# lukifer23/Matrix0

Measured on AMD Instinct MI355X. Metric: self-play games/sec at 800 sims/move, ResNet-24 53M; 1/2/4/8 MI355X, higher is better.
Workload: dtype f16

## Files before the change

### matrix0_amd/csrc/conv_gemm.hip

```cpp
#include "kernel_common.h"
#include "conv_epilogue.h"

template <int TAPS, int WN, int NT, int KC, ConvEpi EPI = EPI_ELEMENT, int ACT = ACT_NONE>
__global__ __launch_bounds__(256 * WN) void conv_gemm_kernel(GemmArgs a) {
    constexpr int NB = WN * NT * 32;
    constexpr int NTHR = 256 * WN;
    constexpr int AST = KC + 8;
    constexpr int APIX = (TAPS == 9) ? 100 : 64;
    constexpr int A_ELEMS = 4 * APIX * AST;
    constexpr int W_ELEMS = NB * AST;
    constexpr int A_PIECES = 4 * 64 * KC / 8;
    constexpr int W_PIECES = NB * KC / 8;
    constexpr int A_PER = (A_PIECES + NTHR - 1) / NTHR;
    constexpr int W_PER = (W_PIECES + NTHR - 1) / NTHR;
    constexpr int K8 = KC / 8;

    extern __shared__ __attribute__((aligned(16))) char smem[];
    _Float16* A_lds = reinterpret_cast<_Float16*>(smem);
    _Float16* W_lds = A_lds + A_ELEMS;

    const int tid = threadIdx.x;
    const int lane = tid & 63;
    const int wave = tid >> 6;
    const int wm = wave % 4;
    const int wn = wave / 4;
    const int m0 = blockIdx.x * 256;
    const int n0 = blockIdx.y * NB;
    const int Cin = a.Cin;
    const int nchunk = Cin / KC;
    const int Npad = a.Npad;

    if (TAPS == 9) {
        for (int i = tid; i < A_ELEMS / 8; i += NTHR)
            reinterpret_cast<uint4*>(A_lds)[i] = make_uint4(0, 0, 0, 0);
    }
    __syncthreads();

    float16v acc[2][NT];
    static_for<0, 2>([&](auto mi) __attribute__((always_inline)) {
        static_for<0, NT>([&](auto ni) __attribute__((always_inline)) {
            acc[decltype(mi)::value][decltype(ni)::value] = float16v{0.f, 0.f, 0.f, 0.f, 0.f, 0.f, 0.f, 0.f,
                                                                      0.f, 0.f, 0.f, 0.f, 0.f, 0.f, 0.f, 0.f};
        });
    });

    int apix[2];
#pragma unroll
    for (int mi = 0; mi < 2; ++mi) {
        int px = mi * 32 + (lane & 31);
        if (TAPS == 9) apix[mi] = wm * 100 + ((px >> 3) + 1) * 10 + (px & 7) + 1;
        else apix[mi] = wm * 64 + px;
    }
    const int khalf = 8 * (lane >> 5);

    uint4 areg[A_PER];
    uint4 wreg[W_PER];

    auto load_A = [&](int chunk) {
#pragma unroll
        for (int i = 0; i < A_PER; ++i) {
            int p = tid + i * NTHR;
            if (A_PIECES % NTHR == 0 || p < A_PIECES) {
                int row = p / K8, c8 = p % K8;
                areg[i] = *reinterpret_cast<const uint4*>(a.in + (size_t)(m0 + row) * Cin + chunk * KC + c8 * 8);
            }
        }
    };
    auto store_A = [&](int chunk) {
#pragma unroll
        for (int i = 0; i < A_PER; ++i) {
            int p = tid + i * NTHR;
            if (A_PIECES % NTHR == 0 || p < A_PIECES) {
                int row = p / K8, c8 = p % K8;
                int b = row >> 6, px = row & 63;
                uint4 v = areg[i];
                int pix = (TAPS == 9) ? (b * 100 + ((px >> 3) + 1) * 10 + (px & 7) + 1) : row;
                *reinterpret_cast<uint4*>(A_lds + pix * AST + c8 * 8) = v;
            }
        }
    };
    auto load_W = [&](int step) {
        int chunk = step / TAPS, tap = step % TAPS;
        const _Float16* src = a.w + ((size_t)(tap * nchunk + chunk) * Npad + n0) * KC;
#pragma unroll
        for (int i = 0; i < W_PER; ++i) {
            int p = tid + i * NTHR;
            if (W_PIECES % NTHR == 0 || p < W_PIECES)
                wreg[i] = *reinterpret_cast<const uint4*>(src + (size_t)p * 8);
        }
    };
    auto store_W = [&](int buf) {
#pragma unroll
        for (int i = 0; i < W_PER; ++i) {
            int p = tid + i * NTHR;
            if (W_PIECES % NTHR == 0 || p < W_PIECES) {
                int n = p / K8, k8 = p % K8;
                *reinterpret_cast<uint4*>(W_lds + buf * W_ELEMS + n * AST + k8 * 8) = wreg[i];
            }
        }
    };

    const int nsteps = nchunk * TAPS;
    load_A(0);
    load_W(0);
    for (int s = 0; s < nsteps; ++s) {
        const int chunk = s / TAPS, tap = s % TAPS;
        if (tap == 0) {
            if (s > 0) __syncthreads();
            store_A(chunk);
        }
        store_W(s & 1);
        __syncthreads();
        if (s + 1 < nsteps) {
            load_W(s + 1);
            if ((s + 1) % TAPS == 0) load_A((s + 1) / TAPS);
        }
        const int tapoff = (TAPS == 9) ? ((tap / 3 - 1) * 10 + (tap % 3 - 1)) : 0;
        const _Float16* Wb = W_lds + (s & 1) * W_ELEMS + (wn * NT * 32 + (lane & 31)) * AST + khalf;
        static_for<0, KC / 16>([&](auto kk_) __attribute__((always_inline)) {
            constexpr int kk = decltype(kk_)::value;
            half8 af0 = *reinterpret_cast<const half8*>(A_lds + (apix[0] + tapoff) * AST + kk * 16 + khalf);
            half8 af1 = *reinterpret_cast<const half8*>(A_lds + (apix[1] + tapoff) * AST + kk * 16 + khalf);
            static_for<0, NT>([&](auto ni_) __attribute__((always_inline)) {
                constexpr int ni = decltype(ni_)::value;
                half8 bf = *reinterpret_cast<const half8*>(Wb + ni * 32 * AST + kk * 16);
                acc[0][ni] = __builtin_amdgcn_mfma_f32_32x32x16_f16(af0, bf, acc[0][ni], 0, 0, 0);
                acc[1][ni] = __builtin_amdgcn_mfma_f32_32x32x16_f16(af1, bf, acc[1][ni], 0, 0, 0);
            });
        });
    }

    if constexpr (EPI == EPI_GN) {
        __syncthreads();
        GemmArgs o = a;
        int out_col0 = 0;
        if (a.out2 != nullptr && n0 + wn * NT * 32 >= a.nsplit) { o.out = a.out2; o.ldo = a.ldo2; out_col0 = a.nsplit; }
        conv_tile_epilogue<EPI_GN, ACT, NT>(acc, o, smem + wave * (64 * 64 * NT), m0, n0, wm, wn, lane, out_col0);
    } else {
        conv_tile_epilogue<EPI_ELEMENT, ACT_NONE, NT>(acc, a, smem, m0, n0, wm, wn, lane);
    }
}

template <int TAPS, int WN, int NT, int KC>
static size_t conv_gemm_lds() {
    constexpr int NB = WN * NT * 32;
    constexpr int AST = KC + 8;
    constexpr int APIX = (TAPS == 9) ? 100 : 64;
    const size_t main_loop = (size_t)(4 * APIX * AST + 2 * NB * AST) * 2 + 64;
    const size_t staging = (size_t)WN * 4 * 64 * 64 * NT;
    return main_loop > staging ? main_loop : staging;
}

template <int TAPS, int WN, int NT, int KC, ConvEpi EPI = EPI_ELEMENT, int ACT = ACT_NONE>
static hipError_t launch_conv_gemm_t(const GemmArgs& a, hipStream_t st) {
    constexpr int NB = WN * NT * 32;
    size_t lds = conv_gemm_lds<TAPS, WN, NT, KC>();
    static DeviceOnce once;
    hipError_t e = once.run([] {
        return hipFuncSetAttribute(reinterpret_cast<const void*>(&conv_gemm_kernel<TAPS, WN, NT, KC, EPI, ACT>),
                                   hipFuncAttributeMaxDynamicSharedMemorySize, 160 * 1024);
    });
    if (e != hipSuccess) return e;
    dim3 grid(a.Mrows / 256, a.Npad / NB);
    hipLaunchKernelGGL((conv_gemm_kernel<TAPS, WN, NT, KC, EPI, ACT>), grid, dim3(256 * WN), lds, st, a);
    return hipGetLastError();
}
template <int ACT>
static hipError_t launch_conv_gemm_gn(const GemmArgs& a, int taps, hipStream_t st) {
    if (a.bias != nullptr || a.mul != nullptr || a.out_stats != nullptr || a.out_f32 || a.out_scale != 1.f || a.Npad != a.N)
        return hipErrorInvalidValue;
    if (taps == 9) return a.Npad % 64 == 0 && a.out2 == nullptr ? launch_conv_gemm_t<9, 1, 2, 32, EPI_GN, ACT>(a, st) : hipErrorInvalidValue;
    if (a.posenc != nullptr) return hipErrorInvalidValue;
    if (a.out2 != nullptr) return a.Npad == 192 && a.nsplit == 64 ? launch_conv_gemm_t<1, 3, 2, 32, EPI_GN, ACT>(a, st) : hipErrorInvalidValue;
    if (a.Npad == 160) return launch_conv_gemm_t<1, 1, 5, 32, EPI_GN, ACT>(a, st);
    if (a.Npad == 128) return launch_conv_gemm_t<1, 2, 2, 32, EPI_GN, ACT>(a, st);
    if (a.Npad == 64) return launch_conv_gemm_t<1, 1, 2, 32, EPI_GN, ACT>(a, st);
    if (a.Npad == 32) return launch_conv_gemm_t<1, 1, 1, 32, EPI_GN, ACT>(a, st);
    return hipErrorInvalidValue;
}

hipError_t launch_conv_big(const GemmArgs& a, int taps, hipStream_t st);
hipError_t launch_conv_zs(const GemmArgs& a, hipStream_t st);

int conv_gemm_tile_n(int Cin, int Npad) {
    return (Npad % 320 == 0 && Cin % 64 == 0) ? 320 : 32;
}
int conv_gemm_kc(int Cin, int Npad) {
    return (Npad % 320 == 0 && Cin % 64 == 0) ? 64 : 32;
}

hipError_t launch_conv_gemm(const GemmArgs& a, int taps, hipStream_t st) {
    if (a.Mrows % 256 != 0 || a.Cin % 32 != 0 || a.Npad % 32 != 0) return hipErrorInvalidValue;
    const bool big = conv_gemm_tile_n(a.Cin, a.Npad) == 320;
    if (a.gn_gamma != nullptr && !big) {
        if (a.epi_act == ACT_SILU) return launch_conv_gemm_gn<ACT_SILU>(a, taps, st);
        if (a.epi_act == ACT_RELU) return launch_conv_gemm_gn<ACT_RELU>(a, taps, st);
        return hipErrorInvalidValue;
    }
    if (taps == 9) {
        if (big) {
            if (!a.w_pp) return hipErrorInvalidValue;
            return launch_conv_zs(a, st);
        }
        return launch_conv_gemm_t<9, 1, 1, 32>(a, st);
    } else if (taps == 1) {
        if (big) return a.w_pp ? hipErrorInvalidValue : launch_conv_big(a, 1, st);
        if (a.Mrows / 256 >= 256 && a.Npad % 64 == 0) return launch_conv_gemm_t<1, 1, 2, 32>(a, st);
        return launch_conv_gemm_t<1, 1, 1, 32>(a, st);
    }
    return hipErrorInvalidValue;
}
```

### matrix0_amd/csrc/net.h

```cpp
#pragma once
#include <hip/hip_runtime.h>
#include <stdint.h>
#include <map>
#include <string>
#include <vector>
#include "../../include/m0_engine.h"
#include "net_kernels.h"

struct HostTensor {
    std::vector<float> data;
    std::vector<int64_t> shape;
};

struct PackedGemm {
    _Float16* w = nullptr;
    float* bias = nullptr;
    int taps = 1, Cin = 0, N = 0;
    bool pp = false;
};

struct NormParams {
    float* gamma = nullptr;
    float* beta = nullptr;
};

struct ResBlockW {
    PackedGemm conv1, conv2;
    NormParams bn1, bn2;
    float *se_w1 = nullptr, *se_b1 = nullptr, *se_w2 = nullptr, *se_b2 = nullptr;
    void* se_wf = nullptr;
    int se_hidden = 0;
};

struct AttnW {
    PackedGemm qkv, proj;
    NormParams ln;
    float* rel_bias = nullptr;
    void* blk_w = nullptr;
    _Float16* blk_bias = nullptr;
};

struct TowerLayer {
    int kind;
    int index;
    bool skip;
    int next_bn1 = -1;
};

struct SslHeadW {
    PackedGemm c0, c1;
    NormParams n;
    int out_ch = 0;
};

struct ConvNormOpts {
    const float* posenc = nullptr;
    const _Float16* res = nullptr;
    const NormParams* next_bn1 = nullptr;
};

class Net {
public:
    explicit Net(const m0_net_cfg& cfg, int device, hipStream_t stream);
    ~Net();
    Net* shared_view(hipStream_t stream) const;
    static const char* check_supported(const m0_net_cfg& cfg);
    int load(const char* name, const void* data, int dtype, const int64_t* shape, int ndim, std::string& err);
    int finalize(std::string& err);
    bool ready() const { return finalized_; }
    const std::vector<void*>& device_buffers() const { return dev_allocs_; }
    const std::vector<size_t>& device_buffer_bytes() const { return dev_sizes_; }

    int forward(const float* planes_dev, const _Float16* nhwc_dev, int B, float* logits_dev, float* value_dev,
                float* ssl_dev, hipStream_t st, std::string& err);
    int ensure_workspace(int B, std::string& err);
    int ssl_channels_total() const;
    const m0_net_cfg& cfg() const { return cfg_; }
    size_t param_count() const { return nparams_; }
    double flops_per_position(bool with_ssl) const;
    _Float16* input_nhwc() { return X0_; }
    void set_profile(bool on) { profile_ = on; }
    void harvest_profile();
    double prof_conv_ms() const { return prof_ms_; }
    double prof_conv_flop() const { return prof_flop_; }
    long prof_conv_launches() const { return prof_launches_; }
    void reset_profile() { prof_ms_ = 0; prof_flop_ = 0; prof_launches_ = 0; prof_tail_ms_ = 0; prof_tail_launches_ = 0; }
    double prof_tail_ms() const { return prof_tail_ms_; }
    long prof_tail_launches() const { return prof_tail_launches_; }

private:
    m0_net_cfg cfg_;
    int device_;
    hipStream_t stream_ = nullptr;
    struct Switches { bool fuse_tail = true, fuse_attn = true; int attn_grid = 0; } sw_;
    struct Plan {
        bool fuse_tail = false;
        bool fuse_attn = false;
        bool gn_small = false;
        int act = 0, vact = 0;
        int first_bn1 = -1;
    } plan_;
    bool finalized_ = false;
    size_t nparams_ = 0;
    std::map<std::string, HostTensor> sd_;
    std::vector<void*> dev_allocs_;
    std::vector<size_t> dev_sizes_;
    std::vector<void*> ws_allocs_;

    int C_ = 0, Cs_ = 0 ;
    int Cp_ = 0;
    PackedGemm stem_;
    NormParams stem_n_;
    float* posenc_ = nullptr;
    PackedGemm pst_, inter_;
    NormParams pst_n_, inter_n_;
    std::vector<ResBlockW> res_;
    std::vector<AttnW> att_;
    std::vector<TowerLayer> tower_;
    PackedGemm ph_conv_, pfc1_, pfc2_;
    PackedGemm hv_;
    NormParams hv_n_;
    NormParams ph_n_;
    float logit_scale_ = 1.f;
    PackedGemm vh0_, vh3_, vfc1_, vfc2_, vgate_, vfc3_;
    NormParams vh1_n_, vh4_n_;
    std::vector<SslHeadW> ssl_;
    uint64_t* mask_dev_ = nullptr;

    bool profile_ = false;
    std::vector<hipEvent_t> pev_;
    std::vector<double> pflop_;
    std::vector<char> ptail_;
    size_t pev_used_ = 0;
    double prof_ms_ = 0, prof_flop_ = 0, prof_tail_ms_ = 0;
    long prof_launches_ = 0, prof_tail_launches_ = 0;

    int wsB_ = 0, wsM_ = 0;
    _Float16 *X0_ = nullptr, *XA_ = nullptr, *XB_ = nullptr, *T1_ = nullptr, *T2_ = nullptr, *QKV_ = nullptr,
             *O_ = nullptr, *AA_ = nullptr;
    float *S1_ = nullptr, *S2_ = nullptr, *G_ = nullptr;
    _Float16 *PH_ = nullptr, *PH2_ = nullptr, *VH_ = nullptr, *VH2_ = nullptr, *F1_ = nullptr, *F2_ = nullptr,
             *F3_ = nullptr, *F4_ = nullptr, *SH_ = nullptr, *SH2_ = nullptr, *SO_ = nullptr;
    float* VAL_ = nullptr;
    float* SPK_ = nullptr;

    const HostTensor* get(const std::string& k, std::string& err);
    int pack_gemm(PackedGemm& g, const std::string& wkey, const std::string& bkey, int taps, int Cin_real,
                  int Cin_pad, int N_real, int N_pad, int k_perm_ch, std::string& err, int qkv_heads = 0,
                  int qkv_heads_pad = 0);
    int pack_attn_block(AttnW& a, const std::string& prefix, std::string& err);
    int pack_chess_features(std::string& err);
    int pack_se(ResBlockW& r, const std::string& prefix, std::string& err);
    int pack_attn(AttnW& a, bool skip, const std::string& prefix, std::string& err);
    void upload_attn_mask();
    int pack_joint_head(std::string& err);
    int pack_ssl_heads(std::string& err);
    void make_plan();
    int upload_norm(NormParams& n, const std::string& prefix, int C_real, int C_pad, std::string& err);
    float* upload_f32(const std::vector<float>& v);
    void* dalloc(size_t bytes, bool ws);
    const NormParams* bn1(int res_index) const { return res_index < 0 ? nullptr : &res_[res_index].bn1; }
    template <class Launch>
    hipError_t profiled(bool on, hipStream_t st, double flop, bool tail, Launch&& launch);
    hipError_t run_gemm(const PackedGemm& g, GemmArgs a, hipStream_t st);
    hipError_t conv_norm_act(const PackedGemm& g, const NormParams& n, const _Float16* in, _Float16* out, _Float16* scratch,
                             int Mrows, hipStream_t st, const ConvNormOpts& o = ConvNormOpts());
    hipError_t se_gate(const ResBlockW& r, const float* stats, int boards, hipStream_t st);
};
```

### matrix0_amd/csrc/net.hip

```cpp
#include "net.h"
#include "attn_math.h"
#include <math.h>
#include <string.h>
#include <algorithm>
#include <stdlib.h>

static inline int ceil_to(int v, int m) { return (v + m - 1) / m * m; }

static const char* kSslNames[5] = {"piece", "threat", "pin", "fork", "control"};
static const int kSslOut[5] = {13, 1, 1, 1, 3};

const char* Net::check_supported(const m0_net_cfg& c) {
    if (!c.norm_group) return "HIP path supports norm='group' only (BatchNorm configs are not built)";
    if (!c.preact) return "HIP path supports preact=true only";
    if (c.channels % 32 != 0 || c.channels < 32 || c.channels > 384) return "channels must be a multiple of 32 in [32,384]";
    if (c.planes < 1 || c.planes > 32) return "planes must be in [1,32]";
    if (c.attention && (c.attention_heads <= 0 || c.channels % c.attention_heads != 0 ||
                        c.channels / c.attention_heads != 16))
        return "attention head_dim (channels/attention_heads) must be 16";
    if (c.activation != M0_ACT_SILU && c.activation != M0_ACT_RELU) return "activation must be silu or relu";
    if (c.blocks < 1) return "blocks must be >= 1";
    if (c.policy_factor_rank < 0) return "policy_factor_rank must be >= 0";
    if (c.self_supervised && c.ssl_tasks && (c.channels / 2) % 16 != 0) return "ssl heads need channels/2 % 16 == 0";
    return nullptr;
}

Net::Net(const m0_net_cfg& cfg, int device, hipStream_t stream) : cfg_(cfg), device_(device), stream_(stream) {
    auto off = [](const char* name) { const char* e = getenv(name); return e && e[0] == '0'; };
    sw_.fuse_tail = !off("M0_FUSE_TAIL");
    sw_.fuse_attn = !off("M0_FUSE_ATTN");
    if (const char* e = getenv("M0_ATTN_GRID")) sw_.attn_grid = std::max(0, atoi(e));
    C_ = cfg.channels;
    Cp_ = (C_ > 256 && C_ < 320) ? 320 : C_;
    Cs_ = ceil_to(std::max(16, C_ / 2), 32);
    int k = cfg.attention_every_k;
    int stride = std::max(1, cfg.infer_attention_stride);
    int att_seen = 0;
    for (int i = 0; i < cfg.blocks; ++i) {
        tower_.push_back({0, (int)res_.size(), false});
        res_.emplace_back();
        if (cfg.attention && k > 0 && (i % k) == (k - 1)) {
            ++att_seen;
            bool skip = stride > 1 && (att_seen % stride) != 0;
            tower_.push_back({1, (int)att_.size(), skip});
            att_.emplace_back();
        }
    }
}

Net* Net::shared_view(hipStream_t stream) const {
    Net* v = new Net(*this);
    v->stream_ = stream;
    v->dev_allocs_.clear(); v->dev_sizes_.clear();
    v->ws_allocs_.clear(); v->wsB_ = 0; v->wsM_ = 0;
    v->sd_.clear();
    v->pev_.clear(); v->pflop_.clear(); v->ptail_.clear(); v->pev_used_ = 0; v->profile_ = false;
    v->prof_ms_ = v->prof_flop_ = v->prof_tail_ms_ = 0; v->prof_launches_ = v->prof_tail_launches_ = 0;
    return v;
}

Net::~Net() {
    for (hipEvent_t e : pev_) (void)hipEventDestroy(e);
    for (void* p : dev_allocs_) (void)hipFree(p);
    for (void* p : ws_allocs_) (void)hipFree(p);
}

void* Net::dalloc(size_t bytes, bool ws) {
    void* p = nullptr;
    if (bytes == 0) bytes = 16;
    if (hipMalloc(&p, bytes) != hipSuccess) return nullptr;
    (void)hipMemsetAsync(p, 0, bytes, stream_);
    if (!ws) (void)hipStreamSynchronize(stream_);
    (ws ? ws_allocs_ : dev_allocs_).push_back(p);
    if (!ws) dev_sizes_.push_back(bytes);
    return p;
}

float* Net::upload_f32(const std::vector<float>& v) {
    float* d = (float*)dalloc(v.size() * 4, false);
    if (d && !v.empty()) (void)hipMemcpy(d, v.data(), v.size() * 4, hipMemcpyHostToDevice);
    return d;
}

int Net::load(const char* name, const void* data, int dtype, const int64_t* shape, int ndim, std::string& err) {
    if (finalized_) { err = "weights already finalized"; return M0_ERR_STATE; }
    if (!name || (!data && ndim >= 0)) { err = "null argument"; return M0_ERR_INVALID; }
    HostTensor t;
    size_t n = 1;
    for (int i = 0; i < ndim; ++i) { t.shape.push_back(shape[i]); n *= (size_t)shape[i]; }
    t.data.resize(n);
    if (dtype == 0) memcpy(t.data.data(), data, n * 4);
    else if (dtype == 1) {
        const _Float16* h = (const _Float16*)data;
        for (size_t i = 0; i < n; ++i) t.data[i] = (float)h[i];
    } else { err = "dtype must be 0 (f32) or 1 (f16)"; return M0_ERR_INVALID; }
    std::string key(name);
    if (cfg_.policy_factor_rank > 0 && key.rfind("policy_fc.", 0) == 0) key = "policy_fc1." + key.substr(10);
    sd_[key] = std::move(t);
    return M0_OK;
}

const HostTensor* Net::get(const std::string& k, std::string& err) {
    auto it = sd_.find(k);
    if (it == sd_.end()) { err = "missing state-dict key: " + k; return nullptr; }
    return &it->second;
}

int Net::pack_gemm(PackedGemm& g, const std::string& wkey, const std::string& bkey, int taps, int Cin_real,
                   int Cin_pad, int N_real, int N_pad, int k_perm_ch, std::string& err, int qkv_heads, int qkv_heads_pad) {
    const HostTensor* w = get(wkey, err);
    if (!w) return M0_ERR_INVALID;
    size_t expect = (size_t)N_real * Cin_real * taps;
    if (w->data.size() != expect) { err = "shape mismatch for " + wkey; return M0_ERR_INVALID; }
    nparams_ += expect;
    const int KC = conv_gemm_kc(Cin_pad, N_pad);
    const int nchunk = Cin_pad / KC;
    const bool pp = KC == 64 && taps == 9;
    const int nblk = N_pad / 320;
    std::vector<_Float16> p((size_t)taps * Cin_pad * N_pad, (_Float16)0.f);
    for (int nr = 0; nr < N_real; ++nr)
        for (int k = 0; k < Cin_real; ++k)
            for (int t = 0; t < taps; ++t) {
                float v = w->data[((size_t)nr * Cin_real + k) * taps + t];
                int n = nr;
                if (qkv_heads > 0) {
                    const int d = nr % 16, th = nr / 16, hh = th % qkv_heads, tt = th / qkv_heads;
                    n = (tt * qkv_heads_pad + hh) * 16 + d;
                }
                int kk = k;
                if (k_perm_ch > 0) {
                    int c = k / 64, sq = k % 64;
                    kk = sq * k_perm_ch + c;
                }
                int chunk = kk / KC, kc = kk % KC;
                if (pp) {
                    const int kt = chunk * 9 + t, by = n / 320, nl = n % 320, h = kc >> 5, k32 = kc & 31;
                    const int kx = (((k32 >> 3) ^ ((4 - ((nl >> 2) & 3)) & 3)) << 3) | (k32 & 7);
                    p[((((size_t)kt * nblk + by) * 2 + h) * 320 + nl) * 32 + kx] = (_Float16)v;
                    continue;
                }
                if (KC == 64)
                    kc = (((kc >> 3) ^ ((n >> 1) & 7)) << 3) | (kc & 7);
                p[(((size_t)t * nchunk + chunk) * N_pad + n) * KC + kc] = (_Float16)v;
            }
    g.w = (_Float16*)dalloc(p.size() * 2, false);
    if (!g.w) { err = "hipMalloc failed"; return M0_ERR_HIP; }
    (void)hipMemcpy(g.w, p.data(), p.size() * 2, hipMemcpyHostToDevice);
    g.taps = taps; g.Cin = Cin_pad; g.N = N_pad; g.pp = pp;
    g.bias = nullptr;
    if (!bkey.empty()) {
        const HostTensor* b = get(bkey, err);
        if (!b) return M0_ERR_INVALID;
        if ((int)b->data.size() != N_real) { err = "shape mismatch for " + bkey; return M0_ERR_INVALID; }
        nparams_ += N_real;
        std::vector<float> bp(N_pad, 0.f);
        std::copy(b->data.begin(), b->data.end(), bp.begin());
        g.bias = upload_f32(bp);
    }
    return M0_OK;
}

int Net::pack_attn_block(AttnW& a, const std::string& prefix, std::string& err) {
    const HostTensor* wq = get(prefix + ".qkv.weight", err); if (!wq) return M0_ERR_INVALID;
    const HostTensor* wp = get(prefix + ".proj.weight", err); if (!wp) return M0_ERR_INVALID;
    const int Cr = C_, Hr = cfg_.attention_heads;
    if (Cp_ != 320 || Cr != Hr * 16 || wq->data.size() != (size_t)3 * Cr * Cr || wp->data.size() != (size_t)Cr * Cr) {
        err = "shape mismatch for " + prefix; return M0_ERR_INVALID;
    }
    std::vector<_Float16> buf(attn_block_pack_bytes() / 2, (_Float16)0.f);
    auto qkv_w = [&](int type, int h, int d, int k) -> float {
        return (h < Hr && k < Cr) ? wq->data[(size_t)((type * Hr + h) * 16 + d) * Cr + k] : 0.f;
    };
    auto proj_w = [&](int oc, int h, int d) -> float {
        return (oc < Cr && h < Hr) ? wp->data[(size_t)oc * Cr + h * 16 + d] : 0.f;
    };
    for (int g = 0; g < 10; ++g) {
        for (int pc = 0; pc < 5; ++pc) {
            const size_t base = (size_t)(g * 7 + pc) * 6144;
            for (int col = 0; col < 96; ++col) {
                const int J = col >> 4, type = J >> 1, hl = J & 1, d = col & 15;
                for (int k = 0; k < 64; ++k) {
                    const int pos = (k >> 3) ^ ((col >> 1) & 7);
                    buf[base + (size_t)col * 64 + pos * 8 + (k & 7)] = (_Float16)qkv_w(type, 2 * g + hl, d, 64 * pc + k);
                }
            }
        }
        for (int hh = 0; hh < 2; ++hh) {
            const size_t base = (size_t)(g * 7 + 5 + hh) * 6144;
            for (int cl = 0; cl < 160; ++cl)
                for (int k = 0; k < 32; ++k) {
                    const int pos = (k >> 3) ^ ((4 - ((cl >> 2) & 3)) & 3);
                    buf[base + (size_t)cl * 32 + pos * 8 + (k & 7)] = (_Float16)proj_w(160 * hh + cl, 2 * g + (k >> 4), k & 15);
                }
        }
    }
    a.blk_w = dalloc(buf.size() * 2, false);
    if (!a.blk_w) { err = "hipMalloc failed"; return M0_ERR_HIP; }
    (void)hipMemcpy(a.blk_w, buf.data(), buf.size() * 2, hipMemcpyHostToDevice);
    std::vector<_Float16> bb((size_t)20 * 2 * 64 * 32, (_Float16)0.f);
    if (cfg_.attention_relbias) {
        const HostTensor* rb = get(prefix + ".rel_bias", err); if (!rb) return M0_ERR_INVALID;
// ... 84 lines not shown
                    for (int e = 0; e < 8; ++e) {
                        const int j = 32 * ks + 8 * (l >> 4) + e, c = 16 * nt + (l & 15);
                        if (j < hd) wf[((size_t)(10 * NT1 + nt * KS2 + ks) * 64 + l) * 8 + e] = (_Float16)w2t[(size_t)j * P + c];
                    }
        r.se_wf = dalloc(wf.size() * 2, false);
        if (!r.se_wf) { err = "hipMalloc failed"; return M0_ERR_HIP; }
        (void)hipMemcpy(r.se_wf, wf.data(), wf.size() * 2, hipMemcpyHostToDevice);
    }
    std::vector<float> b2p(P, 0.f);
    std::copy(b2->data.begin(), b2->data.end(), b2p.begin());
    r.se_b2 = upload_f32(b2p);
    return M0_OK;
}

int Net::pack_attn(AttnW& a, bool skip, const std::string& p, std::string& err) {
    const int C = C_, P = Cp_;
    if (skip) {
        for (const char* k : {".qkv.weight", ".proj.weight", ".norm.weight", ".norm.bias", ".rel_bias"}) {
            auto it = sd_.find(p + k);
            if (it != sd_.end()) nparams_ += it->second.data.size();
        }
        return M0_OK;
    }
    TRY(pack_gemm(a.qkv, p + ".qkv.weight", "", 1, C, P, 3 * C, 3 * P, 0, err, P != C ? cfg_.attention_heads : 0, P / 16));
    TRY(pack_gemm(a.proj, p + ".proj.weight", "", 1, C, P, C, P, 0, err));
    TRY(upload_norm(a.ln, p + ".norm", C, P, err));
    if (P == 320) TRY(pack_attn_block(a, p, err));
    if (cfg_.attention_relbias) {
        const HostTensor* rb = get(p + ".rel_bias", err); if (!rb) return M0_ERR_INVALID;
        if ((int)rb->data.size() != cfg_.attention_heads * 4096) { err = "shape mismatch for rel_bias"; return M0_ERR_INVALID; }
        nparams_ += rb->data.size();
        std::vector<float> rbs((size_t)(P / 16) * 4096, 0.f);
        for (size_t i = 0; i < rb->data.size(); ++i) rbs[i] = rb->data[i] * kLog2e;
        a.rel_bias = upload_f32(rbs);
    }
    return M0_OK;
}

void Net::upload_attn_mask() {
    std::vector<uint64_t> m(64, 0);
    for (int i = 0; i < 64; ++i)
        for (int j = 0; j < 64; ++j) {
            int dr = i / 8 - j / 8, dc = i % 8 - j % 8;
            int adr = abs(dr), adc = abs(dc);
            bool vis = dr == 0 || dc == 0 || adr == adc || (adr == 2 && adc == 1) || (adr == 1 && adc == 2) ||
                       (adr <= 1 && adc <= 1);
            if (vis) m[i] |= (1ull << j);
        }
    mask_dev_ = (uint64_t*)dalloc(64 * 8, false);
    (void)hipMemcpy(mask_dev_, m.data(), 64 * 8, hipMemcpyHostToDevice);
}

int Net::pack_joint_head(std::string& err) {
    const int nch = Cp_ / 32;
    std::vector<_Float16> a((size_t)nch * 64 * 32), b((size_t)nch * 128 * 32), c((size_t)nch * 192 * 32);
    (void)hipMemcpy(a.data(), ph_conv_.w, a.size() * 2, hipMemcpyDeviceToHost);
    (void)hipMemcpy(b.data(), vh0_.w, b.size() * 2, hipMemcpyDeviceToHost);
    for (int ch = 0; ch < nch; ++ch) {
        std::copy(a.begin() + (size_t)ch * 64 * 32, a.begin() + (size_t)(ch + 1) * 64 * 32, c.begin() + (size_t)ch * 192 * 32);
        std::copy(b.begin() + (size_t)ch * 128 * 32, b.begin() + (size_t)(ch + 1) * 128 * 32, c.begin() + ((size_t)ch * 192 + 64) * 32);
    }
    hv_.w = (_Float16*)dalloc(c.size() * 2, false);
    if (!hv_.w) { err = "hipMalloc failed"; return M0_ERR_HIP; }
    (void)hipMemcpy(hv_.w, c.data(), c.size() * 2, hipMemcpyHostToDevice);
    hv_.taps = 1; hv_.Cin = Cp_; hv_.N = 192; hv_.pp = false; hv_.bias = nullptr;
    std::vector<float> g(192), be(192);
    (void)hipMemcpy(g.data(), ph_n_.gamma, 64 * 4, hipMemcpyDeviceToHost);
    (void)hipMemcpy(g.data() + 64, vh1_n_.gamma, 128 * 4, hipMemcpyDeviceToHost);
    (void)hipMemcpy(be.data(), ph_n_.beta, 64 * 4, hipMemcpyDeviceToHost);
    (void)hipMemcpy(be.data() + 64, vh1_n_.beta, 128 * 4, hipMemcpyDeviceToHost);
    hv_n_.gamma = upload_f32(g); hv_n_.beta = upload_f32(be);
    if (!hv_n_.gamma || !hv_n_.beta) { err = "hipMalloc failed"; return M0_ERR_HIP; }
    return M0_OK;
}

int Net::pack_ssl_heads(std::string& err) {
    for (int t = 0; t < 5; ++t) {
        if (!(cfg_.ssl_tasks & (1 << t))) continue;
        SslHeadW h;
        h.out_ch = kSslOut[t];
        std::string p = std::string("ssl_heads.") + kSslNames[t];
        TRY(pack_gemm(h.c0, p + ".0.weight", "", 1, C_, Cp_, C_ / 2, Cs_, 0, err));
        TRY(upload_norm(h.n, p + ".1", C_ / 2, Cs_, err));
        TRY(pack_gemm(h.c1, p + ".3.weight", "", 1, C_ / 2, Cs_, h.out_ch, 32, 0, err));
        ssl_.push_back(h);
    }
    return M0_OK;
}

void Net::make_plan() {
    const bool big = conv_gemm_tile_n(Cp_, Cp_) == 320;
    plan_.fuse_tail = big && sw_.fuse_tail &&
                      (!cfg_.se || (res_[0].se_hidden <= TAIL_SE_HMAX && res_[0].se_hidden % 4 == 0));
    plan_.fuse_attn = big && sw_.fuse_attn;
    plan_.gn_small = Cp_ % 64 == 0;
    plan_.act = cfg_.activation == M0_ACT_SILU ? ACT_SILU : ACT_RELU;
    plan_.vact = cfg_.value_activation == M0_ACT_SILU ? ACT_SILU : (cfg_.value_activation == M0_ACT_LEAKY ? ACT_LEAKY : ACT_RELU);
    int next = -1;
    for (size_t i = tower_.size(); i-- > 0;) {
        TowerLayer& L = tower_[i];
        if (L.kind == 1 && L.skip) continue;
        L.next_bn1 = next;
        next = L.kind == 0 ? L.index : -1;
    }
    plan_.first_bn1 = next;
}

int Net::finalize(std::string& err) {
    if (finalized_) return M0_OK;
    if (hipSetDevice(device_) != hipSuccess) { err = "hipSetDevice failed"; return M0_ERR_HIP; }
    const int C = C_, P = Cp_;
    nparams_ = 0;
    TRY(pack_gemm(stem_, "stem.0.weight", "", 9, cfg_.planes, 32, C, P, 0, err));
    TRY(upload_norm(stem_n_, "stem.1", C, P, err));
    if (cfg_.chess_features) TRY(pack_chess_features(err));
    int ti = 0;
    for (auto& L : tower_) {
        std::string p = "tower." + std::to_string(ti++);
        if (L.kind == 0) {
            ResBlockW& r = res_[L.index];
            TRY(pack_gemm(r.conv1, p + ".conv1.weight", "", 9, C, P, C, P, 0, err));
            TRY(pack_gemm(r.conv2, p + ".conv2.weight", "", 9, C, P, C, P, 0, err));
            TRY(upload_norm(r.bn1, p + ".bn1", C, P, err));
            TRY(upload_norm(r.bn2, p + ".bn2", C, P, err));
            if (cfg_.se) TRY(pack_se(r, p, err));
        } else {
            TRY(pack_attn(att_[L.index], L.skip, p, err));
        }
    }
    upload_attn_mask();
    TRY(pack_gemm(ph_conv_, "policy_head.0.weight", "", 1, C, P, 64, 64, 0, err));
    TRY(upload_norm(ph_n_, "policy_head.1", 64, 64, err));
    if (cfg_.policy_factor_rank > 0) {
        int r = cfg_.policy_factor_rank, rp = ceil_to(r, 32);
        TRY(pack_gemm(pfc1_, "policy_fc1.weight", "policy_fc1.bias", 1, 4096, 4096, r, rp, 64, err));
        TRY(pack_gemm(pfc2_, "policy_fc2.weight", "policy_fc2.bias", 1, r, rp, M0_POLICY_SIZE, M0_POLICY_SIZE, 0, err));
    } else {
        TRY(pack_gemm(pfc1_, "policy_fc.weight", "policy_fc.bias", 1, 4096, 4096, M0_POLICY_SIZE, M0_POLICY_SIZE, 64, err));
    }
    {
        const HostTensor* ls = get("_policy_logit_scale_raw", err); if (!ls) return M0_ERR_INVALID;
        nparams_ += 1;
        double raw = ls->data.empty() ? 0.0 : ls->data[0];
        double sp = raw > 20.0 ? raw : log1p(exp(raw));
        logit_scale_ = (float)std::min(5.0, sp + 1e-3);
    }
    TRY(pack_gemm(vh0_, "value_head.0.weight", "", 1, C, P, 128, 128, 0, err));
    TRY(upload_norm(vh1_n_, "value_head.1", 128, 128, err));
    TRY(pack_gemm(vh3_, "value_head.3.weight", "", 1, 128, 128, 128, 128, 0, err));
    TRY(upload_norm(vh4_n_, "value_head.4", 128, 128, err));
    TRY(pack_joint_head(err));
    const int h1 = 2 * C, h1p = ceil_to(h1, 32), h2 = C, h2p = ceil_to(C, 32);
    TRY(pack_gemm(vfc1_, "value_fc1.weight", "value_fc1.bias", 1, 8192, 8192, h1, h1p, 128, err));
    TRY(pack_gemm(vfc2_, "value_fc2.weight", "value_fc2.bias", 1, h1, h1p, h2, h2p, 0, err));
    TRY(pack_gemm(vgate_, "value_gate.0.weight", "value_gate.0.bias", 1, h2, h2p, h2, h2p, 0, err));
    TRY(pack_gemm(vfc3_, "value_fc3.weight", "value_fc3.bias", 1, h2, h2p, 1, 32, 0, err));
    if (cfg_.self_supervised) TRY(pack_ssl_heads(err));
    sd_.clear();
    (void)hipDeviceSynchronize();
    make_plan();
    finalized_ = true;
    return M0_OK;
}

int Net::ssl_channels_total() const {
    int n = 0;
    for (auto& h : ssl_) n += h.out_ch;
    return n;
}

double Net::flops_per_position(bool with_ssl) const {
    const double C = C_;
    double mac = 64.0 * cfg_.planes * 9 * C;
    if (cfg_.chess_features) mac += 64.0 * C * C * (cfg_.piece_square_tables ? 1 : 0) + 64.0 * C * C * 9;
    for (auto& L : tower_) {
        if (L.kind == 0) {
            mac += 2 * 64.0 * C * C * 9;
            if (cfg_.se) mac += 2.0 * C * res_[L.index].se_hidden;
        } else if (!L.skip) {
            mac += 64.0 * C * 3 * C + 64.0 * C * C;
            double nb = (cfg_.attention_unmasked_mix > 0.f && cfg_.attention_unmasked_mix < 1.f) ? 2.0 : 1.0;
            mac += 64.0 * 64.0 * C * (1.0 + nb);
        }
    }
    mac += 64.0 * C * 64;
    if (cfg_.policy_factor_rank > 0) mac += 4096.0 * cfg_.policy_factor_rank + (double)cfg_.policy_factor_rank * M0_POLICY_SIZE;
    else mac += 4096.0 * M0_POLICY_SIZE;
    mac += 64.0 * C * 128 + 64.0 * 128 * 128 + 8192.0 * 2 * C + 2.0 * C * C + C * C + C;
    if (with_ssl) for (auto& h : ssl_) mac += 64.0 * C * (C / 2) + 64.0 * (C / 2) * h.out_ch;
    return 2.0 * mac;
}

int Net::ensure_workspace(int B, std::string& err) {
    const int Bp = ceil_to(B, 4);
    const int Mfc = ceil_to(B, 256);
    if (Bp <= wsB_ && Mfc <= wsM_) return M0_OK;
    if (hipSetDevice(device_) != hipSuccess) { err = "hipSetDevice failed"; return M0_ERR_HIP; }
    (void)hipDeviceSynchronize();
    for (void* p : ws_allocs_) (void)hipFree(p);
    ws_allocs_.clear();
    const size_t C = Cp_;
    const size_t nb = Bp, nh = std::max(Bp, Mfc);
    const size_t Cst = std::max<size_t>(C, 128);
    auto H = [&](size_t elems) { return (_Float16*)dalloc(elems * 2, true); };
    auto F = [&](size_t elems) { return (float*)dalloc(elems * 4, true); };
    X0_ = H(nb * 64 * 32);
    XA_ = H(nb * 64 * C); XB_ = H(nb * 64 * C); T1_ = H(nb * 64 * C); T2_ = H(nb * 64 * C); AA_ = H(nb * 64 * C);
    QKV_ = H(nb * 64 * 3 * C); O_ = H(nb * 64 * C);
    S1_ = F(nb * Cst * 2); S2_ = F(nb * Cst * 2); G_ = F(nb * Cst);
    PH_ = H(nh * 64 * 64); PH2_ = H(nh * 64 * 64);
    VH_ = H(nh * 64 * 128); VH2_ = H(nh * 64 * 128);
    const size_t rp = cfg_.policy_factor_rank > 0 ? ceil_to(cfg_.policy_factor_rank, 32) : 32;
    F1_ = H((size_t)Mfc * rp);
    F2_ = H((size_t)Mfc * ceil_to(2 * C_, 32)); F3_ = H((size_t)Mfc * ceil_to(C_, 32)); F4_ = H((size_t)Mfc * ceil_to(C_, 32));
    SH_ = H(nb * 64 * Cs_); SH2_ = H(nb * 64 * Cs_); SO_ = H(nb * 64 * 32);
    VAL_ = F((size_t)Mfc * 32);
    SPK_ = F((size_t)8 * Mfc * ceil_to(2 * C_, 32));
    if (!X0_ || !XA_ || !XB_ || !AA_ || !T1_ || !T2_ || !QKV_ || !O_ || !S1_ || !S2_ || !PH_ || !PH2_ || !VH_ ||
        !VH2_ || !F1_ || !F2_ || !F3_ || !F4_ || !SH_ || !SH2_ || !SO_ || !VAL_ || !SPK_) {
        err = "workspace hipMalloc failed";
        wsB_ = wsM_ = 0;
        return M0_ERR_HIP;
    }
    if (hipStreamSynchronize(stream_) != hipSuccess || hipGetLastError() != hipSuccess) {
        err = "workspace clear failed"; wsB_ = wsM_ = 0; return M0_ERR_HIP;
    }
    wsB_ = Bp; wsM_ = Mfc;
    return M0_OK;
}

static GemmArgs gemm_args(const PackedGemm& g, const _Float16* in, void* out, int Mrows, int epi_act = ACT_NONE) {
    GemmArgs a;
    memset(&a, 0, sizeof(a));
    a.in = in; a.w = g.w; a.out = out; a.bias = g.bias;
    a.Mrows = Mrows; a.Mvalid = Mrows; a.Cin = g.Cin; a.N = g.N; a.Npad = g.N; a.ldo = g.N;
    a.epi_act = epi_act; a.out_scale = 1.f; a.w_pp = g.pp ? 1 : 0;
    return a;
}

static EwArgs ew_args(const _Float16* t, _Float16* y, int C, int act) {
    EwArgs e;
    memset(&e, 0, sizeof(e));
    e.t = t; e.y = y; e.C = C; e.act = act;
    return e;
}
static void ew_next_bn1(EwArgs& e, const NormParams* next_bn1, _Float16* y2) {
    if (next_bn1) { e.y2 = y2; e.gn2_gamma = next_bn1->gamma; e.gn2_beta = next_bn1->beta; }
}

static double conv3x3_flop(const PackedGemm& g, int rows) { return 2.0 * (double)rows * (double)g.N * (double)g.Cin * 9.0; }

template <class Launch>
hipError_t Net::profiled(bool on, hipStream_t st, double flop, bool tail, Launch&& launch) {
    if (!on) return launch();
    if (pev_used_ + 2 > pev_.size()) {
        for (int i = 0; i < 2; ++i) { hipEvent_t e; if (hipEventCreate(&e) != hipSuccess) return hipErrorOutOfMemory; pev_.push_back(e); }
    }
    (void)hipEventRecord(pev_[pev_used_], st);
    hipError_t rc = launch();
    (void)hipEventRecord(pev_[pev_used_ + 1], st);
    pev_used_ += 2;
    pflop_.push_back(flop);
    ptail_.push_back(tail ? 1 : 0);
    return rc;
}

hipError_t Net::run_gemm(const PackedGemm& g, GemmArgs a, hipStream_t st) {
    const bool big = conv_gemm_tile_n(g.Cin, g.N) == 320;
    const bool splitk = g.taps == 1 && big && g.Cin >= 4096 && (g.Cin >> 6) % 8 == 0 && !a.gn_gamma && !a.mul && !a.out_stats &&
                        !a.out_f32 && a.out_scale == 1.f && SPK_ != nullptr && (size_t)g.N <= (size_t)ceil_to(2 * C_, 32) &&
                        a.Mrows <= wsM_;
    return profiled(profile_ && g.taps == 9 && big, st, conv3x3_flop(g, a.Mvalid), false, [&]() -> hipError_t {
        if (!splitk) return launch_conv_gemm(a, g.taps, st);
        _Float16* out = (_Float16*)a.out;
        const int act = a.epi_act;
        a.out = SPK_; a.bias = nullptr; a.epi_act = ACT_NONE; a.out_f32 = 1; a.ksplit = 8;
        hipError_t rc = launch_conv_gemm(a, g.taps, st);
        return rc != hipSuccess ? rc : launch_splitk_reduce(SPK_, 8, a.Mrows, g.N, g.bias, act, out, st);
    });
}

hipError_t Net::se_gate(const ResBlockW& r, const float* stats, int boards, hipStream_t st) {
    SeGateArgs g;
    g.t_stats = stats; g.w1 = r.se_w1; g.b1 = r.se_b1; g.w2 = r.se_w2; g.b2 = r.se_b2;
    g.gate = G_; g.B = boards; g.C = Cp_; g.hidden = r.se_hidden; g.act = plan_.act;
    return launch_se_gate(g, st);
}

hipError_t Net::conv_norm_act(const PackedGemm& g, const NormParams& n, const _Float16* in, _Float16* out, _Float16* scratch,
                              int Mrows, hipStream_t st, const ConvNormOpts& o) {
    const bool big = conv_gemm_tile_n(g.Cin, g.N) == 320;
    GemmArgs a = gemm_args(g, in, out, Mrows);
    if (big && o.res && plan_.fuse_tail) {
        a.epi_act = plan_.act; a.res = o.res; a.pre_gamma = n.gamma; a.pre_beta = n.beta;
        if (o.next_bn1) { a.y2 = AA_; a.gn_gamma = o.next_bn1->gamma; a.gn_beta = o.next_bn1->beta; }
        return launch_conv_gemm(a, g.taps, st);
    }
    const bool epilogue = big ? g.taps == 9
                              : plan_.gn_small && (g.taps == 9 ? g.Cin == 32 : g.N == 32 || g.N == 64 || g.N == 128 || g.N == 160);
    if (epilogue && !o.res && !o.next_bn1) {
        a.gn_gamma = n.gamma; a.gn_beta = n.beta; a.epi_act = plan_.act; a.posenc = o.posenc;
        return run_gemm(g, a, st);
    }
    a.out = scratch; a.out_stats = S1_;
    hipError_t rc = run_gemm(g, a, st);
    if (rc != hipSuccess) return rc;
    EwArgs e = ew_args(scratch, out, g.N, plan_.act);
    e.t_stats = S1_; e.gn_gamma = n.gamma; e.gn_beta = n.beta; e.res = o.res; e.posenc = o.posenc;
    ew_next_bn1(e, o.next_bn1, AA_);
    return launch_ew_board(e, Mrows / 64, st);
}

void Net::harvest_profile() {
    for (size_t i = 0; i + 1 < pev_used_; i += 2) {
        float ms = 0.f;
        if (hipEventElapsedTime(&ms, pev_[i], pev_[i + 1]) == hipSuccess) {
            prof_ms_ += ms; prof_flop_ += pflop_[i / 2]; prof_launches_++;
            if (ptail_[i / 2]) { prof_tail_ms_ += ms; prof_tail_launches_++; }
        }
    }
    pev_used_ = 0;
// ... 138 lines not shown
```

### matrix0_amd/csrc/net_kernels.h

```cpp
#pragma once
#include <hip/hip_runtime.h>
#include <stdint.h>

enum { ACT_NONE = 0, ACT_RELU = 1, ACT_SILU = 2, ACT_LEAKY = 3, ACT_SIGMOID = 4, ACT_TANH = 5 };

enum ConvEpi {
    EPI_PLAIN,
    EPI_GN,
    EPI_ELEMENT,
    EPI_TAIL,
    EPI_TAIL_PRE,
};

constexpr int TAIL_SE_HMAX = 96;

struct GemmArgs {
    const _Float16* in;
    const _Float16* w;
    void* out;
    const float* gn_gamma;
    const float* gn_beta;
    const float* bias;
    const _Float16* mul;
    float* out_stats;
    int Mrows;
    int Mvalid;
    int Cin;
    int N;
    int Npad;
    int ldo;
    int epi_act;
    int out_f32;
    float out_scale;
    int ksplit;
    int w_pp;
    const _Float16* res;
    const float* pre_gamma;
    const float* pre_beta;
    _Float16* y2;
    const float* se_w1;
    const float* se_b1;
    const float* se_w2;
    const float* se_b2;
    int se_hidden;
    const void* se_wf;
    const float* posenc;
    void* out2;
    int ldo2;
    int nsplit;
};

struct EwArgs {
    const _Float16* t;
    const float* t_stats;
    const float* gn_gamma;
    const float* gn_beta;
    const float* gate;
    const _Float16* res;
    const float* posenc;
    const float* ln_g;
    const float* ln_b;
    int ln_count;
    _Float16* y;
    float* out_stats;
    _Float16* y2;
    const float* gn2_gamma;
    const float* gn2_beta;
    int C;
    int act;
};

struct SeGateArgs {
    const float* t_stats;
    const float* w1;
    const float* b1;
    const float* w2;
    const float* b2;
    float* gate;
    int B, C, hidden, act;
};
// ... 43 lines not shown
```

Before: 1.165.

## Add dedicated stem conv kernel and K-chunk-64 paths for head GEMMs

```diff
diff --git a/matrix0_amd/csrc/conv_gemm.hip b/matrix0_amd/csrc/conv_gemm.hip
--- a/matrix0_amd/csrc/conv_gemm.hip
+++ b/matrix0_amd/csrc/conv_gemm.hip
@@ -53,8 +53,8 @@
     }
     const int khalf = 8 * (lane >> 5);
 
-    uint4 areg[A_PER];
-    uint4 wreg[W_PER];
+    half8 areg[A_PER];
+    half8 wreg[W_PER];
 
     auto load_A = [&](int chunk) {
 #pragma unroll
@@ -62,7 +62,7 @@
             int p = tid + i * NTHR;
             if (A_PIECES % NTHR == 0 || p < A_PIECES) {
                 int row = p / K8, c8 = p % K8;
-                areg[i] = *reinterpret_cast<const uint4*>(a.in + (size_t)(m0 + row) * Cin + chunk * KC + c8 * 8);
+                areg[i] = *reinterpret_cast<const half8*>(a.in + (size_t)(m0 + row) * Cin + chunk * KC + c8 * 8);
             }
         }
     };
@@ -73,9 +73,9 @@
             if (A_PIECES % NTHR == 0 || p < A_PIECES) {
                 int row = p / K8, c8 = p % K8;
                 int b = row >> 6, px = row & 63;
-                uint4 v = areg[i];
+                half8 v = areg[i];
                 int pix = (TAPS == 9) ? (b * 100 + ((px >> 3) + 1) * 10 + (px & 7) + 1) : row;
-                *reinterpret_cast<uint4*>(A_lds + pix * AST + c8 * 8) = v;
+                *reinterpret_cast<half8*>(A_lds + pix * AST + c8 * 8) = v;
             }
         }
     };
@@ -86,7 +86,7 @@
         for (int i = 0; i < W_PER; ++i) {
             int p = tid + i * NTHR;
             if (W_PIECES % NTHR == 0 || p < W_PIECES)
-                wreg[i] = *reinterpret_cast<const uint4*>(src + (size_t)p * 8);
+                wreg[i] = *reinterpret_cast<const half8*>(src + (size_t)p * 8);
         }
     };
     auto store_W = [&](int buf) {
@@ -95,7 +95,7 @@
             int p = tid + i * NTHR;
             if (W_PIECES % NTHR == 0 || p < W_PIECES) {
                 int n = p / K8, k8 = p % K8;
-                *reinterpret_cast<uint4*>(W_lds + buf * W_ELEMS + n * AST + k8 * 8) = wreg[i];
+                *reinterpret_cast<half8*>(W_lds + buf * W_ELEMS + n * AST + k8 * 8) = wreg[i];
             }
         }
     };
@@ -166,14 +166,136 @@
     return hipGetLastError();
 }
 template <int ACT>
+__global__ __launch_bounds__(256, 2) void conv_stem_kernel(GemmArgs a) {
+    constexpr int NT = 2, NB = 64, KC = 32, AST = KC + 8;
+    constexpr int A_ELEMS = 4 * 100 * AST;
+    constexpr int W_ELEMS = 9 * NB * AST;
+    static_assert(4 * 64 * 64 * NT <= W_ELEMS * 2, "staging images over the weight slices");
+
+    extern __shared__ __attribute__((aligned(16))) char smem[];
+    _Float16* A_lds = reinterpret_cast<_Float16*>(smem);
+    _Float16* W_lds = A_lds + A_ELEMS;
+
+    const int tid = threadIdx.x;
+    const int lane = tid & 63;
+    const int wm = tid >> 6;
+    const int m0 = blockIdx.x * 256;
+    const int Npad = a.Npad;
+    const int nblk = Npad / NB;
+
+    half8 wreg[9];
+    auto load_W = [&](int nb) __attribute__((always_inline)) {
+        static_for<0, 9>([&](auto t_) __attribute__((always_inline)) {
+            constexpr int t = decltype(t_)::value;
+            wreg[t] = *reinterpret_cast<const half8*>(a.w + ((size_t)t * Npad + nb * NB) * KC + (size_t)tid * 8);
+        });
+    };
+    auto store_W = [&]() __attribute__((always_inline)) {
+        static_for<0, 9>([&](auto t_) __attribute__((always_inline)) {
+            constexpr int t = decltype(t_)::value;
+            *reinterpret_cast<half8*>(W_lds + (t * NB + (tid >> 2)) * AST + (tid & 3) * 8) = wreg[t];
+        });
+    };
+
+    half8 areg[4];
+    static_for<0, 4>([&](auto i_) __attribute__((always_inline)) {
+        constexpr int i = decltype(i_)::value;
+        const int p = tid + i * 256;
+        areg[i] = *reinterpret_cast<const half8*>(a.in + (size_t)(m0 + (p >> 2)) * KC + (p & 3) * 8);
+    });
+    load_W(0);
+    for (int i = tid; i < A_ELEMS / 8; i += 256) reinterpret_cast<uint4*>(A_lds)[i] = make_uint4(0, 0, 0, 0);
+    __syncthreads();
+    static_for<0, 4>([&](auto i_) __attribute__((always_inline)) {
+        constexpr int i = decltype(i_)::value;
+        const int p = tid + i * 256;
+        const int row = p >> 2, b = row >> 6, px = row & 63;
+        *reinterpret_cast<half8*>(A_lds + (b * 100 + ((px >> 3) + 1) * 10 + (px & 7) + 1) * AST + (p & 3) * 8) = areg[i];
+    });
+    store_W();
+    __syncthreads();
+
+    int apix[2];
+#pragma unroll
+    for (int mi = 0; mi < 2; ++mi) {
+        const int px = mi * 32 + (lane & 31);
+        apix[mi] = wm * 100 + ((px >> 3) + 1) * 10 + (px & 7) + 1;
+    }
+    const int khalf = 8 * (lane >> 5);
+    char* stage = reinterpret_cast<char*>(W_lds) + wm * (64 * 64 * NT);
+
+    for (int nb = 0; nb < nblk; ++nb) {
+        const bool more = nb + 1 < nblk;
+        if (more) load_W(nb + 1);
+        float16v acc[2][NT];
+        static_for<0, 2>([&](auto mi) __attribute__((always_inline)) {
+            static_for<0, NT>([&](auto ni) __attribute__((always_inline)) {
+                acc[decltype(mi)::value][decltype(ni)::value] = float16v{0.f, 0.f, 0.f, 0.f, 0.f, 0.f, 0.f, 0.f,
+                                                                          0.f, 0.f, 0.f, 0.f, 0.f, 0.f, 0.f, 0.f};
+            });
+        });
+#pragma unroll 1
+        for (int ty = 0; ty < 3; ++ty) {
+            static_for<0, 3>([&](auto tx_) __attribute__((always_inline)) {
+                constexpr int tx = decltype(tx_)::value;
+                const int tapoff = (ty - 1) * 10 + (tx - 1);
+                const _Float16* Wb = W_lds + ((ty * 3 + tx) * NB + (lane & 31)) * AST + khalf;
+                static_for<0, KC / 16>([&](auto kk_) __attribute__((always_inline)) {
+                    constexpr int kk = decltype(kk_)::value;
+                    half8 af0 = *reinterpret_cast<const half8*>(A_lds + (apix[0] + tapoff) * AST + kk * 16 + khalf);
+                    half8 af1 = *reinterpret_cast<const half8*>(A_lds + (apix[1] + tapoff) * AST + kk * 16 + khalf);
+                    static_for<0, NT>([&](auto ni_) __attribute__((always_inline)) {
+                        constexpr int ni = decltype(ni_)::value;
+                        half8 bf = *reinterpret_cast<const half8*>(Wb + ni * 32 * AST + kk * 16);
+                        acc[0][ni] = __builtin_amdgcn_mfma_f32_32x32x16_f16(af0, bf, acc[0][ni], 0, 0, 0);
+                        acc[1][ni] = __builtin_amdgcn_mfma_f32_32x32x16_f16(af1, bf, acc[1][ni], 0, 0, 0);
+                    });
+                });
+            });
+        }
+        __syncthreads();
+        int elane = lane;
+        asm volatile("" : "+v"(elane));
+        conv_tile_epilogue<EPI_GN, ACT, NT>(acc, a, stage, m0, nb * NB, wm, 0, elane);
+        if (more) {
+            __syncthreads();
+            store_W();
+            __syncthreads();
+        }
+    }
+}
+
+template <int ACT>
+static hipError_t launch_conv_stem(const GemmArgs& a, hipStream_t st) {
+    const size_t lds = (size_t)(4 * 100 + 9 * 64) * 40 * 2;
+    static DeviceOnce once;
+    hipError_t e = once.run([] {
+        return hipFuncSetAttribute(reinterpret_cast<const void*>(&conv_stem_kernel<ACT>),
+                                   hipFuncAttributeMaxDynamicSharedMemorySize, 160 * 1024);
+    });
+    if (e != hipSuccess) return e;
+    hipLaunchKernelGGL((conv_stem_kernel<ACT>), dim3(a.Mrows / 256), dim3(256), lds, st, a);
+    return hipGetLastError();
+}
+
+template <int ACT>
 static hipError_t launch_conv_gemm_gn(const GemmArgs& a, int taps, hipStream_t st) {
     if (a.bias != nullptr || a.mul != nullptr || a.out_stats != nullptr || a.out_f32 || a.out_scale != 1.f || a.Npad != a.N)
         return hipErrorInvalidValue;
-    if (taps == 9) return a.Npad % 64 == 0 && a.out2 == nullptr ? launch_conv_gemm_t<9, 1, 2, 32, EPI_GN, ACT>(a, st) : hipErrorInvalidValue;
+    const bool kc64 = a.kc == 64;
+    if (taps == 9) {
+        if (kc64 || a.Npad % 64 != 0 || a.out2 != nullptr) return hipErrorInvalidValue;
+        if (a.edge && a.Cin == 32 && a.Npad == 320) return launch_conv_stem<ACT>(a, st);
+        return launch_conv_gemm_t<9, 1, 2, 32, EPI_GN, ACT>(a, st);
+    }
     if (a.posenc != nullptr) return hipErrorInvalidValue;
-    if (a.out2 != nullptr) return a.Npad == 192 && a.nsplit == 64 ? launch_conv_gemm_t<1, 3, 2, 32, EPI_GN, ACT>(a, st) : hipErrorInvalidValue;
+    if (a.out2 != nullptr) {
+        if (a.Npad != 192 || a.nsplit != 64) return hipErrorInvalidValue;
+        return kc64 ? launch_conv_gemm_t<1, 3, 2, 64, EPI_GN, ACT>(a, st) : launch_conv_gemm_t<1, 3, 2, 32, EPI_GN, ACT>(a, st);
+    }
+    if (kc64) return hipErrorInvalidValue;
+    if (a.Npad == 128) return launch_conv_gemm_t<1, 2, 2, 32, EPI_GN, ACT>(a, st);
     if (a.Npad == 160) return launch_conv_gemm_t<1, 1, 5, 32, EPI_GN, ACT>(a, st);
-    if (a.Npad == 128) return launch_conv_gemm_t<1, 2, 2, 32, EPI_GN, ACT>(a, st);
     if (a.Npad == 64) return launch_conv_gemm_t<1, 1, 2, 32, EPI_GN, ACT>(a, st);
     if (a.Npad == 32) return launch_conv_gemm_t<1, 1, 1, 32, EPI_GN, ACT>(a, st);
     return hipErrorInvalidValue;
@@ -192,6 +314,7 @@
 hipError_t launch_conv_gemm(const GemmArgs& a, int taps, hipStream_t st) {
     if (a.Mrows % 256 != 0 || a.Cin % 32 != 0 || a.Npad % 32 != 0) return hipErrorInvalidValue;
     const bool big = conv_gemm_tile_n(a.Cin, a.Npad) == 320;
+    if (big ? a.kc != 0 && a.kc != 64 : a.kc != 0 && a.kc != 32 && (a.kc != 64 || a.Cin % 64 != 0)) return hipErrorInvalidValue;
     if (a.gn_gamma != nullptr && !big) {
         if (a.epi_act == ACT_SILU) return launch_conv_gemm_gn<ACT_SILU>(a, taps, st);
         if (a.epi_act == ACT_RELU) return launch_conv_gemm_gn<ACT_RELU>(a, taps, st);
@@ -202,9 +325,10 @@
             if (!a.w_pp) return hipErrorInvalidValue;
             return launch_conv_zs(a, st);
         }
-        return launch_conv_gemm_t<9, 1, 1, 32>(a, st);
+        return a.kc == 64 ? hipErrorInvalidValue : launch_conv_gemm_t<9, 1, 1, 32>(a, st);
     } else if (taps == 1) {
         if (big) return a.w_pp ? hipErrorInvalidValue : launch_conv_big(a, 1, st);
+        if (a.kc == 64) return launch_conv_gemm_t<1, 1, 1, 64>(a, st);
         if (a.Mrows / 256 >= 256 && a.Npad % 64 == 0) return launch_conv_gemm_t<1, 1, 2, 32>(a, st);
         return launch_conv_gemm_t<1, 1, 1, 32>(a, st);
     }
diff --git a/matrix0_amd/csrc/net.h b/matrix0_amd/csrc/net.h
--- a/matrix0_amd/csrc/net.h
+++ b/matrix0_amd/csrc/net.h
@@ -16,6 +16,7 @@
     _Float16* w = nullptr;
     float* bias = nullptr;
     int taps = 1, Cin = 0, N = 0;
+    int kc = 0;
     bool pp = false;
 };
 
@@ -92,7 +93,7 @@
     m0_net_cfg cfg_;
     int device_;
     hipStream_t stream_ = nullptr;
-    struct Switches { bool fuse_tail = true, fuse_attn = true; int attn_grid = 0; } sw_;
+    struct Switches { bool fuse_tail = true, fuse_attn = true, edge = true; int attn_grid = 0; } sw_;
     struct Plan {
         bool fuse_tail = false;
         bool fuse_attn = false;
@@ -147,7 +148,8 @@
     const HostTensor* get(const std::string& k, std::string& err);
     int pack_gemm(PackedGemm& g, const std::string& wkey, const std::string& bkey, int taps, int Cin_real,
                   int Cin_pad, int N_real, int N_pad, int k_perm_ch, std::string& err, int qkv_heads = 0,
-                  int qkv_heads_pad = 0);
+                  int qkv_heads_pad = 0, int kc = 0);
+    int edge_kc() const { return sw_.edge && Cp_ == 320 ? 64 : 32; }
     int pack_attn_block(AttnW& a, const std::string& prefix, std::string& err);
     int pack_chess_features(std::string& err);
     int pack_se(ResBlockW& r, const std::string& prefix, std::string& err);
diff --git a/matrix0_amd/csrc/net.hip b/matrix0_amd/csrc/net.hip
--- a/matrix0_amd/csrc/net.hip
+++ b/matrix0_amd/csrc/net.hip
@@ -29,6 +29,7 @@
     auto off = [](const char* name) { const char* e = getenv(name); return e && e[0] == '0'; };
     sw_.fuse_tail = !off("M0_FUSE_TAIL");
     sw_.fuse_attn = !off("M0_FUSE_ATTN");
+    if (const char* e = getenv("M0_EDGE_GENERIC")) sw_.edge = e[0] != '1';
     if (const char* e = getenv("M0_ATTN_GRID")) sw_.attn_grid = std::max(0, atoi(e));
     C_ = cfg.channels;
     Cp_ = (C_ > 256 && C_ < 320) ? 320 : C_;
@@ -107,15 +108,17 @@
 }
 
 int Net::pack_gemm(PackedGemm& g, const std::string& wkey, const std::string& bkey, int taps, int Cin_real,
-                   int Cin_pad, int N_real, int N_pad, int k_perm_ch, std::string& err, int qkv_heads, int qkv_heads_pad) {
+                   int Cin_pad, int N_real, int N_pad, int k_perm_ch, std::string& err, int qkv_heads, int qkv_heads_pad, int kc) {
     const HostTensor* w = get(wkey, err);
     if (!w) return M0_ERR_INVALID;
     size_t expect = (size_t)N_real * Cin_real * taps;
     if (w->data.size() != expect) { err = "shape mismatch for " + wkey; return M0_ERR_INVALID; }
     nparams_ += expect;
-    const int KC = conv_gemm_kc(Cin_pad, N_pad);
+    const bool big = conv_gemm_tile_n(Cin_pad, N_pad) == 320;
+    const int KC = (kc > 0 && !big) ? kc : conv_gemm_kc(Cin_pad, N_pad);
+    if (Cin_pad % KC != 0) { err = "K chunk does not divide Cin for " + wkey; return M0_ERR_INVALID; }
     const int nchunk = Cin_pad / KC;
-    const bool pp = KC == 64 && taps == 9;
+    const bool pp = big && taps == 9;
     const int nblk = N_pad / 320;
     std::vector<_Float16> p((size_t)taps * Cin_pad * N_pad, (_Float16)0.f);
     for (int nr = 0; nr < N_real; ++nr)
@@ -139,14 +142,14 @@
                     p[((((size_t)kt * nblk + by) * 2 + h) * 320 + nl) * 32 + kx] = (_Float16)v;
                     continue;
                 }
-                if (KC == 64)
+                if (big)
                     kc = (((kc >> 3) ^ ((n >> 1) & 7)) << 3) | (kc & 7);
                 p[(((size_t)t * nchunk + chunk) * N_pad + n) * KC + kc] = (_Float16)v;
             }
     g.w = (_Float16*)dalloc(p.size() * 2, false);
     if (!g.w) { err = "hipMalloc failed"; return M0_ERR_HIP; }
     (void)hipMemcpy(g.w, p.data(), p.size() * 2, hipMemcpyHostToDevice);
-    g.taps = taps; g.Cin = Cin_pad; g.N = N_pad; g.pp = pp;
+    g.taps = taps; g.Cin = Cin_pad; g.N = N_pad; g.pp = pp; g.kc = KC;
     g.bias = nullptr;
     if (!bkey.empty()) {
         const HostTensor* b = get(bkey, err);
@@ -337,18 +340,19 @@
 }
 
 int Net::pack_joint_head(std::string& err) {
-    const int nch = Cp_ / 32;
+    const int nch = Cp_ / 32, KC = edge_kc(), per = KC / 32;
     std::vector<_Float16> a((size_t)nch * 64 * 32), b((size_t)nch * 128 * 32), c((size_t)nch * 192 * 32);
     (void)hipMemcpy(a.data(), ph_conv_.w, a.size() * 2, hipMemcpyDeviceToHost);
     (void)hipMemcpy(b.data(), vh0_.w, b.size() * 2, hipMemcpyDeviceToHost);
-    for (int ch = 0; ch < nch; ++ch) {
-        std::copy(a.begin() + (size_t)ch * 64 * 32, a.begin() + (size_t)(ch + 1) * 64 * 32, c.begin() + (size_t)ch * 192 * 32);
-        std::copy(b.begin() + (size_t)ch * 128 * 32, b.begin() + (size_t)(ch + 1) * 128 * 32, c.begin() + ((size_t)ch * 192 + 64) * 32);
-    }
+    for (int ch = 0; ch < nch; ++ch)
+        for (int n = 0; n < 192; ++n) {
+            const _Float16* src = n < 64 ? &a[((size_t)ch * 64 + n) * 32] : &b[((size_t)ch * 128 + n - 64) * 32];
+            std::copy(src, src + 32, c.begin() + ((size_t)(ch / per) * 192 + n) * KC + (ch % per) * 32);
+        }
     hv_.w = (_Float16*)dalloc(c.size() * 2, false);
     if (!hv_.w) { err = "hipMalloc failed"; return M0_ERR_HIP; }
     (void)hipMemcpy(hv_.w, c.data(), c.size() * 2, hipMemcpyHostToDevice);
-    hv_.taps = 1; hv_.Cin = Cp_; hv_.N = 192; hv_.pp = false; hv_.bias = nullptr;
+    hv_.taps = 1; hv_.Cin = Cp_; hv_.N = 192; hv_.pp = false; hv_.kc = KC; hv_.bias = nullptr;
     std::vector<float> g(192), be(192);
     (void)hipMemcpy(g.data(), ph_n_.gamma, 64 * 4, hipMemcpyDeviceToHost);
     (void)hipMemcpy(g.data() + 64, vh1_n_.gamma, 128 * 4, hipMemcpyDeviceToHost);
@@ -418,10 +422,11 @@
     TRY(upload_norm(ph_n_, "policy_head.1", 64, 64, err));
     if (cfg_.policy_factor_rank > 0) {
         int r = cfg_.policy_factor_rank, rp = ceil_to(r, 32);
-        TRY(pack_gemm(pfc1_, "policy_fc1.weight", "policy_fc1.bias", 1, 4096, 4096, r, rp, 64, err));
+        TRY(pack_gemm(pfc1_, "policy_fc1.weight", "policy_fc1.bias", 1, 4096, 4096, r, rp, 64, err, 0, 0, edge_kc()));
         TRY(pack_gemm(pfc2_, "policy_fc2.weight", "policy_fc2.bias", 1, r, rp, M0_POLICY_SIZE, M0_POLICY_SIZE, 0, err));
     } else {
-        TRY(pack_gemm(pfc1_, "policy_fc.weight", "policy_fc.bias", 1, 4096, 4096, M0_POLICY_SIZE, M0_POLICY_SIZE, 64, err));
+        TRY(pack_gemm(pfc1_, "policy_fc.weight", "policy_fc.bias", 1, 4096, 4096, M0_POLICY_SIZE, M0_POLICY_SIZE, 64, err, 0, 0,
+                      edge_kc()));
     }
     {
         const HostTensor* ls = get("_policy_logit_scale_raw", err); if (!ls) return M0_ERR_INVALID;
@@ -519,7 +524,7 @@
     memset(&a, 0, sizeof(a));
     a.in = in; a.w = g.w; a.out = out; a.bias = g.bias;
     a.Mrows = Mrows; a.Mvalid = Mrows; a.Cin = g.Cin; a.N = g.N; a.Npad = g.N; a.ldo = g.N;
-    a.epi_act = epi_act; a.out_scale = 1.f; a.w_pp = g.pp ? 1 : 0;
+    a.epi_act = epi_act; a.out_scale = 1.f; a.w_pp = g.pp ? 1 : 0; a.kc = g.kc;
     return a;
 }
 
@@ -552,6 +557,7 @@
 
 hipError_t Net::run_gemm(const PackedGemm& g, GemmArgs a, hipStream_t st) {
     const bool big = conv_gemm_tile_n(g.Cin, g.N) == 320;
+    a.edge = sw_.edge ? 1 : 0;
     const bool splitk = g.taps == 1 && big && g.Cin >= 4096 && (g.Cin >> 6) % 8 == 0 && !a.gn_gamma && !a.mul && !a.out_stats &&
                         !a.out_f32 && a.out_scale == 1.f && SPK_ != nullptr && (size_t)g.N <= (size_t)ceil_to(2 * C_, 32) &&
                         a.Mrows <= wsM_;
diff --git a/matrix0_amd/csrc/net_kernels.h b/matrix0_amd/csrc/net_kernels.h
--- a/matrix0_amd/csrc/net_kernels.h
+++ b/matrix0_amd/csrc/net_kernels.h
@@ -26,6 +26,8 @@
     int Mrows;
     int Mvalid;
     int Cin;
+    int kc;
+    int edge;
     int N;
     int Npad;
     int ldo;
```

New measurement: 1.165 (median of 3 runs). Within noise of the previous version (+0.0%).
